# Storm-131/MARL-SortingEnv

Measured on AMD Instinct MI355X. Metric: env-steps/sec (random policy) Env_3_Monolith @65k envs, higher is better.
Workload: dtype int32+f64 (integer state/masks, fp64 rewards, f32 observations)

## Files before the change

__graft_entry__.py:

```python
from __future__ import annotations

import os
import sys

ROOT = os.path.dirname(os.path.abspath(__file__))
if ROOT not in sys.path:
    sys.path.insert(0, ROOT)


def build() -> None:
    import marl_sortingenv_amd as M

    path = M.build_library(force=False)
    assert os.path.exists(path), path
    from marl_sortingenv_amd.build import build_widetie_library

    wide = build_widetie_library()
    assert os.path.exists(wide), wide
    L = M.load_library()
    assert L.mse_version() == 200
    from oracle import oracle as O

    O.build()
    O.lib()
    print(f"built {path} and {O._SO}")


def smoke() -> None:
    import numpy as np
    import torch

    import marl_sortingenv_amd as M
    from oracle.oracle import OracleEnv

    assert torch.cuda.is_available(), "smoke() needs a GPU"
    n, K = 96, 24
    env = M.BatchedSortingEnv(kind="mono", num_envs=n, device=0, base_seed=11, max_steps=10, noise_sorting=0.05,
                              balesize=200, auto_reset=True)
    oracles = [OracleEnv(kind="mono", max_steps=10, seed=11 + i, noise_sorting=0.05, balesize=200) for i in range(n)]
    for i, o in enumerate(oracles):
        assert np.array_equal(env.obs[i].cpu().numpy(), o.reset(11 + i))
    buf = env.rollout(K, policy_seed=5)
    torch.cuda.synchronize()
    act, obs, rew = buf["actions"].cpu().numpy(), buf["obs"].cpu().numpy(), buf["reward"].cpu().numpy()
    done, mask = buf["done"].cpu().numpy(), buf["mask"].cpu().numpy()
    for k in range(K):
        for i, o in enumerate(oracles):
            assert o.action_masks()[act[k, i]] == 1
            eo, er, et = o.step(int(act[k, i]))
            if et:
                eo = o.reset(None)
            assert np.array_equal(eo.view(np.uint32), obs[k, i].view(np.uint32)), (k, i)
            assert abs(er - float(rew[k, i])) <= 1e-6 and bool(done[k, i]) == et
            assert np.array_equal(o.action_masks(), mask[k, i])
    print(f"smoke ok: {n} envs x {K} steps on {torch.cuda.get_device_name(0)} match the oracle "
          f"(lib: {M.library_path()})")


if __name__ == "__main__":
    build()
    if len(sys.argv) > 1 and sys.argv[1] == "smoke":
        smoke()
```

include/mse.h:

```cpp
#ifndef MSE_H
#define MSE_H

#include <stddef.h>
#include <stdint.h>

#ifdef __cplusplus
extern "C" {
#endif

#define MSE_VERSION 200

typedef enum mse_status {
    MSE_OK = 0,
    MSE_ERR_INVALID_ARGUMENT = -1,
    MSE_ERR_UNSUPPORTED_CONFIG = -2,
    MSE_ERR_NO_DEVICE = -3,
    MSE_ERR_HIP = -4,
    MSE_ERR_NOT_RESET = -5,
    MSE_ERR_ALIGNMENT = -6
} mse_status;

typedef enum mse_env_kind { MSE_ENV_SORT = 1, MSE_ENV_PRESS = 2, MSE_ENV_MONO = 3 } mse_env_kind;

#define MSE_STEP_UNMASKED       1u
// ... 66 lines not shown

int mse_rollout(mse_env *env, int32_t k_steps, uint64_t policy_seed, const int32_t *sort_mode_dev,
                uint32_t flags, int32_t *actions_out, float *obs_out, float *reward_out,
                uint8_t *done_out, uint8_t *mask_out, void *stream);

int mse_sample_actions(mse_env *env, uint64_t policy_seed, int32_t *action_out, void *stream);

int mse_rule_actions(mse_env *env, int32_t *action_out, void *stream);

#define MSE_SNAP_INTS 71
#define MSE_SNAP_RNG_WORDS 30
int mse_get_state(mse_env *env, int64_t *ints_out, double *dbls_out, uint64_t *rng_out, void *stream);
int mse_set_state(mse_env *env, const int64_t *ints_in, const double *dbls_in, const uint64_t *rng_in, void *stream);

int mse_model_actions(mse_env *env, uint32_t flags, int32_t *action_out, void *stream);

#define MSE_MODEL_PRESS_AGENT_MASKED 64u
struct mse_policy;
int mse_rollout_model(mse_env *env, struct mse_policy *sort_agent, struct mse_policy *press_agent, int32_t k_steps, uint32_t flags,
                      int32_t *actions_out, float *obs_out, float *reward_out, uint8_t *done_out, uint8_t *mask_out,
                      float *sort_obs_out, float *press_obs_out, void *stream);

#define MSE_TRACE_COLS       40
#define MSE_TRACE_ACTION      0
#define MSE_TRACE_R_SORT      1
#define MSE_TRACE_R_PRESS     2
#define MSE_TRACE_SETTING     3
#define MSE_TRACE_BELT        4
#define MSE_TRACE_CONT_TRUE   8
#define MSE_TRACE_CONT_FALSE 12
#define MSE_TRACE_CONT_E     16
#define MSE_TRACE_N_LOG      17
#define MSE_TRACE_LOG        18
#define MSE_TRACE_N_BALE     22
#define MSE_TRACE_BALE       23
#define MSE_TRACE_DONE       29
#define MSE_TRACE_STEP       30
#define MSE_TRACE_INTERNAL   31
#define MSE_TRACE_REWARD     32
#define MSE_TRACE_ACC_BELT   33
#define MSE_TRACE_OVERFLOW   37
int mse_trace_begin(mse_env *env, int64_t env_index, double *records_dev, int64_t capacity);
int mse_trace_end(mse_env *env, int64_t *n_records_out);

int mse_get_policy_step(const mse_env *env, uint64_t *t_out);
int mse_set_policy_step(mse_env *env, uint64_t t);

int mse_error_count(mse_env *env, uint64_t *count_out);

int mse_algorithmic_bytes_per_step(const mse_env *env);

uint32_t mse_tie_window(void);

typedef struct mse_policy mse_policy;
int64_t mse_policy_num_weights(int obs_dim, int n_actions);
int mse_policy_create(mse_policy **out, int obs_dim, int n_actions, const float *weights_host, int device_id);
int mse_policy_destroy(mse_policy *policy);
int mse_policy_set_precision(mse_policy *policy, int mode);
int mse_policy_precision(const mse_policy *policy);
int mse_policy_forward(mse_policy *policy, int64_t n, int64_t index_offset, const float *obs_dev, const uint8_t *mask_dev,
                       uint64_t seed, uint64_t t, int deterministic, int32_t *action_out, float *logp_out,
                       float *value_out, float *logits_out, void *stream);

int mse_rollout_policy(mse_env *env, mse_policy *policy, mse_policy *sort_policy, int32_t k_steps, uint64_t seed, int deterministic,
                       const int32_t *sort_mode_dev, uint32_t flags, float *obs_out, uint8_t *mask_out,
                       int32_t *actions_out, float *logp_out, float *value_out, float *reward_out,
                       uint8_t *episode_start_out, float *last_value_out, uint8_t *last_done_out, void *stream);

#define MSE_MODULAR_SORT_DETERMINISTIC  128u
#define MSE_MODULAR_PRESS_DETERMINISTIC 256u
typedef struct mse_modular_buffers {
    uint32_t struct_size;
    uint32_t reserved0;
    float   *sort_obs;
    float   *press_obs;
    uint8_t *press_masks;
    uint8_t *episode_starts;
    int32_t *sort_actions;
    int32_t *press_actions;
    float   *sort_log_probs;
    float   *press_log_probs;
    float   *sort_values;
    float   *press_values;
    float   *rewards;
    float   *rewards_sort;
    float   *rewards_press;
    float   *sort_last_values;
    float   *press_last_values;
    uint8_t *last_dones;
} mse_modular_buffers;
int mse_rollout_modular(mse_env *env, mse_policy *sort_agent, mse_policy *press_agent, int32_t k_steps, uint64_t sort_seed,
                        uint64_t press_seed, uint32_t flags, const mse_modular_buffers *out, void *stream);
int mse_rollout_modular_check(mse_env *env, mse_policy *sort_agent, mse_policy *press_agent, int32_t k_steps,
                              uint64_t sort_seed, uint64_t press_seed, uint32_t flags);

typedef struct mse_modular_label_buffers {
    uint32_t struct_size;
    uint32_t reserved0;
    int32_t *sort_expert_actions;
    int32_t *press_expert_actions;
    int32_t *stepped_actions;
    uint8_t *expert_stepped;
} mse_modular_label_buffers;
int mse_rollout_modular_labelled(mse_env *env, mse_policy *sort_agent, mse_policy *press_agent, int32_t k_steps,
                                 uint64_t sort_seed, uint64_t press_seed, uint64_t mix_seed, uint32_t expert_threshold,
                                 uint32_t flags, const mse_modular_buffers *out, const mse_modular_label_buffers *labels,
// ... 145 lines not shown
```

marl-sortingenv_amd/_lib.py:

```python
from __future__ import annotations

import ctypes as C
import os

from .build import LIB_PATH

MSE_ENV_SORT, MSE_ENV_PRESS, MSE_ENV_MONO = 1, 2, 3
MSE_STEP_UNMASKED, MSE_STEP_CHECK_OVERFLOW, MSE_ROLLOUT_RULE_BASED, MSE_STEP_SANITIZE_LATE = 1, 2, 4, 8
MSE_MODEL_NO_SORT_DRAW, MSE_MODEL_NO_PRESS_DRAW = 16, 32
MSE_MODEL_PRESS_AGENT_MASKED = 64
MSE_MODULAR_SORT_DETERMINISTIC, MSE_MODULAR_PRESS_DETERMINISTIC = 128, 256
MSE_DEMO_ACTOR_DETERMINISTIC = 512
MSE_PREVIEW_DETERMINISTIC = 1024
MSE_SNAP_INTS = 71
MSE_SNAP_RNG_WORDS = 30
MSE_TRACE_COLS = 40

EXPORTS = [
    "mse_version", "mse_last_error", "mse_status_string", "mse_config_default", "mse_create",
    "mse_create_indexed", "mse_destroy", "mse_num_envs", "mse_obs_dim", "mse_num_actions", "mse_reset",
    "mse_step", "mse_action_masks", "mse_rollout", "mse_sample_actions", "mse_rule_actions", "mse_get_state", "mse_set_state",
    "mse_error_count", "mse_algorithmic_bytes_per_step", "mse_tie_window",
    "mse_sort_agent_obs", "mse_policy_num_weights", "mse_policy_create", "mse_policy_destroy", "mse_policy_forward",
    "mse_get_policy_step", "mse_set_policy_step", "mse_model_actions", "mse_trace_begin", "mse_trace_end", "mse_press_agent_obs", "mse_rollout_policy", "mse_policy_set_precision", "mse_policy_precision",
    "mse_rollout_model", "mse_rollout_modular", "mse_rollout_modular_check",
    "mse_policy_set_weights", "mse_gae", "mse_ppo_workspace_bytes", "mse_ppo_loss_grad", "mse_ppo_adam_step",
    "mse_ppo_shuffle", "mse_ppo_shuffle_host",
    "mse_policy_set_weights_device", "mse_policy_sync", "mse_policy_image_floats", "mse_policy_pack_host",
    "mse_policy_read_image", "mse_policy_get_weights", "mse_ppo_loss_grad_gated", "mse_ppo_adam_step_gated",
    "mse_episode_workspace_bytes", "mse_episode_scan", "mse_episode_scan_host", "mse_episode_summary", "mse_episode_summary_host",
    "mse_ppo_loss_grad_matrix",
    "mse_ppo_loss_grad_vclip", "mse_explained_variance_workspace_bytes", "mse_explained_variance", "mse_explained_variance_host",
    "mse_bc_loss_grad", "mse_ppo_bc_workspace_bytes", "mse_ppo_bc_loss_grad",
    "mse_rollout_demo", "mse_rollout_demo_check", "mse_demo_who_steps_host",
    "mse_rollout_policy_labelled", "mse_rollout_policy_labelled_check",
    "mse_rollout_modular_labelled", "mse_rollout_modular_labelled_check",
    "mse_mono_agent_obs", "mse_rollout_policy_preview", "mse_rollout_policy_preview_check",
]

_other_libs: dict = {}


class MseError(RuntimeError):
    def __init__(self, status: int, message: str):
        super().__init__(f"libmse_hip status {status}: {message}")
        self.status = status


class MseConfigStruct(C.Structure):
    _fields_ = [
        ("struct_size", C.c_uint32), ("env_kind", C.c_int32), ("max_steps", C.c_int32),
        ("auto_reset", C.c_int32), ("track_bales", C.c_int32), ("literal_choice", C.c_int32),
        ("input_batch_size", C.c_int32), ("steps_per_pattern", C.c_int32),
        ("baseline_accuracy", C.c_double * 4), ("boost", C.c_double), ("noise", C.c_double),
        ("stage_capacity", C.c_int32),
        ("press_time", C.c_int32 * 2), ("container_capacity", C.c_int32), ("bale_standard_size", C.c_int32),
        ("bale_remainder_threshold", C.c_double), ("quality_threshold", C.c_double * 4),
        ("quality_threshold_r2", C.c_double * 4),
        ("purity_threshold_theta", C.c_double), ("tanh_temperature", C.c_double),
        ("overflow_penalty_catastrophic", C.c_double), ("overflow_penalty_severe", C.c_double),
        ("overflow_penalty_mild", C.c_double), ("bale_efficiency_factor", C.c_double),
        ("max_state_reward", C.c_double), ("overflow_termination_penalty", C.c_double),
        ("pattern_ratio", (C.c_double * 4) * 2),
        ("rollout_pipeline", C.c_int32), ("reserved0", C.c_int32),
    ]


class MsePpoParams(C.Structure):
    _fields_ = [("struct_size", C.c_uint32), ("clip_range", C.c_float), ("ent_coef", C.c_float), ("vf_coef", C.c_float),
                ("normalize_advantage", C.c_int32)]


MODULAR_BUFFER_NAMES = ("sort_obs", "press_obs", "press_masks", "episode_starts", "sort_actions", "press_actions",
                        "sort_log_probs", "press_log_probs", "sort_values", "press_values", "rewards", "rewards_sort",
                        "rewards_press", "sort_last_values", "press_last_values", "last_dones")
# ... 150 lines not shown
```

marl-sortingenv_amd/build.py:

```python
from __future__ import annotations

import os
import shutil
import subprocess

PKG_DIR = os.path.dirname(os.path.abspath(__file__))
REPO_ROOT = os.path.dirname(PKG_DIR)
SOURCES = [os.path.join(PKG_DIR, "csrc", "mse_lib.hip"), os.path.join(PKG_DIR, "csrc", "mse_policy.hip"),
           os.path.join(PKG_DIR, "csrc", "mse_ppo.hip"), os.path.join(PKG_DIR, "csrc", "mse_ppo_matrix.hip"),
           os.path.join(PKG_DIR, "csrc", "mse_episode.hip")]
HEADERS = [os.path.join(PKG_DIR, "csrc", h) for h in ("mse_device.h", "mse_exact.h", "mse_host.h", "mse_params.h", "mse_plan.h", "mse_tables.h", "mse_policy_device.h", "mse_policy_pack.h", "mse_policy_stream.h", "mse_demo_mix.h", "mse_ppo_math.h", "mse_ppo_grad.h", "mse_ppo_grad_body.inc", "mse_ppo_matrix_body.inc", "mse_rollout_policy_body.inc", "mse_rollout_modular_body.inc", "mse_plain_frame.inc", "mse_episode_math.h")] + \
          [os.path.join(REPO_ROOT, "include", "mse.h")]
LIB_PATH = os.environ.get("MSE_LIB_PATH") or os.path.join(PKG_DIR, "libmse_hip.so")

HIPCC_FLAGS = [
    "-O3", "--offload-arch=gfx950", "-std=c++17", "-fPIC", "-shared",
    "-ffp-contract=off", "-fno-fast-math",
]


def hipcc_path() -> str:
    for cand in (shutil.which("hipcc"), "/opt/rocm/bin/hipcc"):
        if cand and os.path.exists(cand):
            return cand
    raise RuntimeError("hipcc not found: libmse_hip.so cannot be built")


def is_stale() -> bool:
    if not os.path.exists(LIB_PATH):
        return True
    t = os.path.getmtime(LIB_PATH)
    return any(os.path.getmtime(p) > t for p in SOURCES + HEADERS)


def build_library(force: bool = False, verbose: bool = False) -> str:
    if not force and not is_stale():
        return LIB_PATH
    cmd = [hipcc_path(), *HIPCC_FLAGS, "-I", os.path.join(REPO_ROOT, "include"), *SOURCES, "-o", LIB_PATH]
    if verbose:
        print(" ".join(cmd))
    subprocess.run(cmd, check=True)
    return LIB_PATH


WIDETIE_LIB_PATH = os.path.join(PKG_DIR, "libmse_hip_widetie.so")


def build_widetie_library(force: bool = False) -> str:
    if not force and os.path.exists(WIDETIE_LIB_PATH) and \
            all(os.path.getmtime(p) <= os.path.getmtime(WIDETIE_LIB_PATH) for p in SOURCES + HEADERS):
        return WIDETIE_LIB_PATH
    cmd = [hipcc_path(), *HIPCC_FLAGS, "-DMSE_TIE_WINDOW=0x08000000u", "-I", os.path.join(REPO_ROOT, "include"),
           *SOURCES, "-o", WIDETIE_LIB_PATH]
    subprocess.run(cmd, check=True)
    return WIDETIE_LIB_PATH


if __name__ == "__main__":
    print(build_widetie_library(force=True))
    print(build_library(force=True, verbose=True))
```

marl-sortingenv_amd/csrc/mse_device.h:

```cpp
#pragma once

#include <hip/hip_runtime.h>
#include <stdint.h>

#include "mse_exact.h"
#include "mse_params.h"
#include "mse_policy_stream.h"

namespace mse {

constexpr int kGeneratorPeriod = 20;

enum Plane : int {
    PL_RNG_STATE = 0,
    PL_RNG_INC,
    PL_ACC01,
    PL_ACC23,
    PL_CONT_TRUE,
    PL_CONT_FALSE,
    PL_MISC0,
    PL_MISC1,
    PL_MISC2,
    PL_NOISE_STATE,
    PL_NOISE_INC,
// ... 143 lines not shown
        hb *= MULT_B;
        v *= hb;
        v ^= v >> 16;
        st[i] = v;
    }
#pragma unroll
    for (int i = 0; i < 4; ++i) out[i] = (uint64_t)st[2 * i] | ((uint64_t)st[2 * i + 1] << 32);
}

__device__ inline Pcg pcg_seed(uint64_t seed)
{
    uint64_t w[4];
    seed_sequence(seed, w);
    Pcg g;
    g.i_hi = (w[2] << 1) | (w[3] >> 63);
    g.i_lo = (w[3] << 1) | 1ull;
    g.s_lo = 0;
    g.s_hi = 0;
    pcg_advance(g);
    uint64_t lo = g.s_lo + w[1];
    g.s_hi = g.s_hi + w[0] + (lo < g.s_lo ? 1ull : 0ull);
    g.s_lo = lo;
    pcg_advance(g);
    return g;
}

__device__ __forceinline__ uint64_t mix64(uint64_t z)
{
    z = (z ^ (z >> 30)) * 0xBF58476D1CE4E5B9ull;
    z = (z ^ (z >> 27)) * 0x94D049BB133111EBull;
    return z ^ (z >> 31);
}

__device__ __forceinline__ int select_kth_bit(uint32_t bits, int k)
{
    uint32_t lo = bits & 0x7FFu;
    int c = __popc(lo);
    bool up = k >= c;
    k = up ? k - c : k;
    bits = up ? bits >> 11 : lo;
    int base = up ? 11 : 0;
    lo = bits & 0x3Fu;
    c = __popc(lo);
    up = k >= c;
    k = up ? k - c : k;
    bits = up ? bits >> 6 : lo;
    base += up ? 6 : 0;
    for (int i = 0; i < k; ++i) bits &= bits - 1u;
    return base + __ffs((int)bits) - 1;
}

#ifdef MSE_TIMELINE
__device__ unsigned long long g_timeline[4 * 8];
struct Timeline {
    unsigned long long last;
    unsigned long long acc[8];
    __device__ __forceinline__ void start()
    {
        for (int k = 0; k < 8; ++k) acc[k] = 0;
        last = __builtin_readcyclecounter();
    }
    __device__ __forceinline__ void mark(int k)
    {
        if (blockIdx.x != 0) return;
        const unsigned long long now = __builtin_readcyclecounter();
        acc[k] += now - last;
        last = now;
    }
    __device__ __forceinline__ void flush(int role) const
    {
        if ((threadIdx.x & 63) == 0 && blockIdx.x == 0)
            for (int k = 0; k < 8; ++k) atomicAdd(&g_timeline[role * 8 + k], acc[k]);
    }
};
#if MSE_TIMELINE == 2
#define MSE_TL(tl, k) ((void)0)
#define MSE_TLB(tl, k) (tl).mark(k)
#else
#define MSE_TL(tl, k) (tl).mark(k)
#define MSE_TLB(tl, k) (tl).mark(k)
#endif
#else
#define MSE_TLB(tl, k) ((void)0)
#define MSE_TL(tl, k) ((void)0)
#endif

struct Env {
#ifdef MSE_TIMELINE
    Timeline tl;
#endif
    Pcg rng;
    Pcg noise;
    Pcg press;
    uint32_t press_uint;
    int press_has;
    Pcg gen;
    uint32_t gen_uint;
    int gen_has;
    double acc[4];
    int ct[4], cf[4], ce;
    int pn[2], lpa;
    int st_in, st_belt, st_sort;
    int timer[2], pmat[2], q100[2];
    int mode, lps, gen2, gen_idx, gen_cnt, step;
    uint32_t episode;
};

__device__ __forceinline__ int stage_id(uint32_t word, const Params &P)
{
    if (P.gen_mode) return (int)word;
    return word == 0u ? 0 : (word == P.pat_word[1] ? 1 : 2);
}
__device__ __forceinline__ uint32_t stage_word(int id, const Params &P)
{
    if (P.gen_mode) return (uint32_t)id;
    return id == 0 ? P.pat_word[0] : (id == 1 ? P.pat_word[1] : P.pat_word[2]);
}

struct EnvRaw {
    uint4 a, b, c0, c1, t, f, m0, m1, m2, ns, nq, ps, pq;
};

template <int KIND, bool NOISE>
__device__ __forceinline__ void load_env_raw(EnvRaw &r, const uint4 *__restrict__ planes, const Params &P, long long i)
{
    const long long n_pad = P.n_pad;
    r.a = planes[PL_RNG_STATE * n_pad + i];
    r.b = planes[PL_RNG_INC * n_pad + i];
    r.c0 = planes[PL_ACC01 * n_pad + i];
    r.c1 = planes[PL_ACC23 * n_pad + i];
    r.t = planes[PL_CONT_TRUE * n_pad + i];
    r.f = planes[PL_CONT_FALSE * n_pad + i];
    r.m0 = planes[PL_MISC0 * n_pad + i];
    r.m1 = planes[PL_MISC1 * n_pad + i];
    r.m2 = planes[PL_MISC2 * n_pad + i];
    if (NOISE) {
        r.ns = planes[PL_NOISE_STATE * n_pad + i];
// ... 1625 lines not shown
```

marl-sortingenv_amd/csrc/mse_lib.hip:

```cpp
#include "mse_device.h"
#include "mse_demo_mix.h"
#include "mse_host.h"
#include "mse_plan.h"
#include "mse_policy_device.h"
#include "mse_tables.h"

#include "mse.h"

#include <cmath>
#include <cstdio>
#include <cstdlib>
#include <cstring>
#include <memory>
#include <new>
#include <string>
#include <type_traits>
#include <vector>

using namespace mse;

extern __shared__ uint4 mse_dyn_lds[];

template <int KIND>
struct LdsLayout {
    static constexpr int D = Dims<KIND>::D, A = Dims<KIND>::A;
    static constexpr int obs_bytes = kBlock * D * 4;
    static constexpr int mask_bytes = (kBlock * A + 15) / 16 * 16;
    static constexpr int bale_offset = obs_bytes + mask_bytes;
    static constexpr int bale_bytes = 5 * kBlock * 16;
    static constexpr int table_offset_step = bale_offset;
    static constexpr int table_offset_rollout = bale_offset + bale_bytes;
};

__device__ __forceinline__ void lds_barrier_all()
{
    asm volatile("s_waitcnt lgkmcnt(0)\n\ts_barrier" ::: "memory");
}

template <int THREADS, int U>
struct TableCopy {
    uint4 x[U];
    __device__ __forceinline__ void issue(const uint32_t *__restrict__ src, int words, int t)
    {
        const uint4 *s4 = reinterpret_cast<const uint4 *>(src);
        const int n4 = words >> 2;
#pragma unroll
        for (int u = 0; u < U; ++u) {
            const int idx = u * THREADS + t;
            x[u] = s4[idx < n4 ? idx : n4 - 1];
        }
    }
    __device__ __forceinline__ void commit(uint32_t *dst, const uint32_t *__restrict__ src, int words, int t) const
    {
        uint4 *d4 = reinterpret_cast<uint4 *>(dst);
        const uint4 *s4 = reinterpret_cast<const uint4 *>(src);
        const int n4 = words >> 2;
#pragma unroll
        for (int u = 0; u < U; ++u) {
            const int idx = u * THREADS + t;
            if (idx < n4) d4[idx] = x[u];
        }
        for (int idx = U * THREADS + t; idx < n4; idx += THREADS) d4[idx] = s4[idx];
    }
};

__device__ __forceinline__ void load_tables_to_lds(uint32_t *dst, const uint32_t *__restrict__ src, int words, int tid)
{
    TableCopy<kBlock, 4> tc;
    tc.issue(src, words, tid);
    tc.commit(dst, src, words, tid);
    __syncthreads();
}

typedef float nt_f32x4 __attribute__((ext_vector_type(4)));
typedef unsigned int nt_u32x4 __attribute__((ext_vector_type(4)));
__device__ __forceinline__ void store_stream(float4 *p, const float4 &v)
{
    nt_f32x4 x = {v.x, v.y, v.z, v.w};
    __builtin_nontemporal_store(x, reinterpret_cast<nt_f32x4 *>(p));
}
__device__ __forceinline__ void store_stream(uint4 *p, const uint4 &v)
{
    nt_u32x4 x = {v.x, v.y, v.z, v.w};
    __builtin_nontemporal_store(x, reinterpret_cast<nt_u32x4 *>(p));
}

typedef uint32_t u32_align2 __attribute__((aligned(2)));
template <int A, class P16>
__device__ __forceinline__ void write_mask_row(P16 *row16, uint32_t mbits)
// ... 465 lines not shown
            Snap sn;
#pragma unroll
            for (int m = 0; m < 4; ++m) {
                sn.ct[m] = (int)w[(kSnapCt + m) * kPoEnvs];
                sn.cf[m] = (int)w[(kSnapCf + m) * kPoEnvs];
            }
            sn.ce = (int)w[kSnapCe * kPoEnvs];
            sn.lpa = (int)w[kSnapLpa * kPoEnvs];
            const uint32_t pk = w[kSnapStatus * kPoEnvs];
            const int a = (int)w[kSnapAction * kPoEnvs];
            const uint32_t mbits = w[kSnapMask * kPoEnvs];
            if (NOISE) {
#pragma unroll
                for (int m = 0; m < 4; ++m)
                    sn.acc[m] = __hiloint2double((int)w[(kSnapAcc + 2 * m + 1) * kPoEnvs], (int)w[(kSnapAcc + 2 * m) * kPoEnvs]);
            }
            unpack_snap_status(pk, sn);
            if (live) {
                int k[4];
                StepResult r = env_observe<KIND, NOISE>(sn, P, tb, k, o);
                if (__builtin_expect(sn.done != 0, 0)) {
                    Snap rs;
                    snap_of_reset(rs, tb.cst);
                    int k2[4];
                    (void)env_observe<KIND, true>(rs, P, tb, k2, o);
                }
                if (actions_out != nullptr) __builtin_nontemporal_store(a, &actions_out[(long long)s * P.n + i]);
                if (reward_out != nullptr) __builtin_nontemporal_store((float)r.reward, &reward_out[(long long)s * P.n + i]);
                if (done_out != nullptr) __builtin_nontemporal_store((uint8_t)r.done, &done_out[(long long)s * P.n + i]);
            }
            const long long srow = (long long)s * P.n + row0;
            stage_and_store<KIND>(lds, L::obs_bytes, o, mbits, obs_out ? obs_out + srow * D : nullptr,
                                  mask_out ? mask_out + srow * A : nullptr, n_valid_block, tid - kPoEnvs);
        }
    }
}

constexpr int kRingThreads = 3 * kPoEnvs;

template <int KIND, bool NOISE>
struct RingLayout {
    static constexpr int D = Dims<KIND>::D, A = Dims<KIND>::A;
    static constexpr int snap_words = snap_word_count(NOISE, false);
    static constexpr int ring_offset = 0;
    static constexpr int ring_bytes = kRingDepth * kPoEnvs * 4;
    static_assert(ring_bytes == 65536, "RngRing::load assumes 64 rows of 1 KiB");
    static constexpr int stage_offset = ring_bytes;
    static constexpr int stage_bytes = kPoEnvs * D * 4;
    static constexpr int snap_offset = stage_offset + stage_bytes;
    static constexpr int snap_bytes = 2 * snap_words * kPoEnvs * 4;
    static constexpr int bale_offset = snap_offset + snap_bytes;
    static constexpr int bale_bytes = 5 * kPoEnvs * 16;
    static constexpr int pos_offset = bale_offset + bale_bytes;
    static constexpr int pos_bytes = kPoEnvs * 4;
    static constexpr int table_offset = pos_offset + pos_bytes;
};

__device__ __forceinline__ void rng_server_role(const Params &P, uint4 *__restrict__ planes, const Tables &tb, long long i,
                                                bool live, int k_steps, uint32_t *lring, uint32_t *lpos, int el, bool two_halves,
                                                int barriers_before_init = 0)
{
    Pcg g = Pcg::from_planes(planes[PL_RNG_STATE * P.n_pad + i], planes[PL_RNG_INC * P.n_pad + i]);
    const uint32_t ring_lane_addr = (uint32_t)(uintptr_t)(__attribute__((address_space(3))) uint32_t *)(lring + el);
    uint64_t c2_lo, c2_hi;
    mul128(0x4385DF649FCCF646ull, 0x2360ED051FC65DA4ull, g.i_lo, g.i_hi, c2_lo, c2_hi);
    const uint32_t worst = (uint32_t)P.ring_worst;
    uint32_t w = 0, need = worst, cap = need;
#ifdef MSE_TIMELINE
    Timeline tl;
    tl.start();
#endif
    for (int s = -1; s < k_steps; ++s) {
        const uint32_t deficit = need > w ? need - w : 0u;
        uint32_t M = 0;
#pragma unroll
        for (int bit = 5; bit >= 0; --bit) {
            const uint32_t cand = M | (1u << bit);
            if (__builtin_amdgcn_ballot_w64(deficit >= cand) != 0ull) M = cand;
        }
        const uint32_t room = cap > w ? cap - w : 0u;
#ifdef MSE_TIMELINE
        if (blockIdx.x == 0) {
            tl.acc[3] += M;
            unsigned long long produced = 0;
            for (int b = 0; b < 6; ++b) produced += ((unsigned long long)__builtin_popcountll(__builtin_amdgcn_ballot_w64((((M < room ? M : room) >> b) & 1u) != 0))) << b;
            tl.acc[4] += produced;
        }
#endif
#ifdef MSE_ABL_NORNG
        w += M < room ? M : room;
#else
        {
            const uint32_t count = M < room ? M : room;
            ring_produce_pairs(g, w, count >> 1, ring_lane_addr, c2_lo, c2_hi);
            ring_produce(g, w, count & 1u, ring_lane_addr);
        }
#endif
        MSE_TLB(tl, 0);
        if (s < 0)
            for (int b = 0; b < barriers_before_init; ++b) lds_barrier_all();
        lds_barrier_all();
        MSE_TLB(tl, 1);
        if (s < 0 && two_halves) {
            pcg_affine(g, P.ring_fwd[0], P.ring_fwd[1], P.ring_fwd[2], P.ring_fwd[3]);
            w += worst;
        }
        const uint32_t steps_left = (uint32_t)(k_steps - 1 - s);
        const uint32_t r = lpos[el];
        const uint32_t ahead = worst * steps_left;
        need = r + worst * (steps_left < 2u ? steps_left : 2u);
        cap = r + (ahead < (uint32_t)kRingDepth ? ahead : (uint32_t)kRingDepth);
    }
    {
        uint32_t d = w - lpos[el];
        if (__builtin_expect(d > 32u, 0)) {
            pcg_step_back(g, 32u, tb.back);
            d -= 32u;
        }
        pcg_step_back(g, d, tb.back);
        if (live) planes[PL_RNG_STATE * P.n_pad + i] = pack_u64x2(g.s_lo, g.s_hi);
    }
#ifdef MSE_TIMELINE
    tl.flush(2);
#endif
}

constexpr int kRingTwoHalvesFrom = 16;

#ifdef MSE_CLOCK_PROBE
__device__ unsigned long long g_clock_probe[3];
__device__ unsigned long long g_wg_probe[3 * 1024];
#endif
template <int KIND, bool NOISE>
__global__ __launch_bounds__(kRingThreads) void k_rollout_ring(Params P, uint4 *__restrict__ planes,
                                                               const uint32_t *__restrict__ table_image, int k_steps,
                                                               uint64_t policy_seed, uint64_t policy_t0,
                                                               const int *__restrict__ sort_mode, uint32_t flags,
                                                               int *__restrict__ actions_out,
                                                               float *__restrict__ obs_out,
                                                               float *__restrict__ reward_out,
                                                               uint8_t *__restrict__ done_out,
                                                               uint8_t *__restrict__ mask_out)
{
    using L = RingLayout<KIND, NOISE>;
    constexpr int D = L::D, A = L::A, SW = L::snap_words;
    uint8_t *lds = reinterpret_cast<uint8_t *>(mse_dyn_lds);
    uint32_t *ltab = reinterpret_cast<uint32_t *>(lds + L::table_offset);
    uint32_t *lsnap = reinterpret_cast<uint32_t *>(lds + L::snap_offset);
    uint4 *lbale = reinterpret_cast<uint4 *>(lds + L::bale_offset);
    uint32_t *lring = reinterpret_cast<uint32_t *>(lds + L::ring_offset);
    uint32_t *lpos = reinterpret_cast<uint32_t *>(lds + L::pos_offset);
    const int tid = threadIdx.x;
    const int role = tid / kPoEnvs;
    const int el = tid - role * kPoEnvs;
    const long long row0 = (long long)blockIdx.x * kPoEnvs;
    const bool live = row0 + el < P.n;
    const long long i = live ? row0 + el : P.n - 1;
#ifdef MSE_TIMELINE
    Timeline edge;
    edge.start();
#endif
#ifdef MSE_CLOCK_PROBE
    const unsigned long long probe_c0 = __builtin_readcyclecounter(), probe_r0 = __builtin_amdgcn_s_memrealtime();
#endif

    const Tables tb = tables_at(ltab, P);
    Env e;
    EnvRaw raw;
    int sm = -1;
    if (role == 0) {
        load_env_raw<KIND, NOISE>(raw, planes, P, i);
        if (KIND == 2 && sort_mode != nullptr) sm = sort_mode[i];
    }
    if (role == 0) {
        TableCopy<2 * kPoEnvs, 2> tc;
        tc.issue(table_image, P.table_words, tid);
        tc.commit(ltab, table_image, P.table_words, tid);
        unpack_env<KIND, NOISE>(e, raw, P);
    } else if (role == 1) {
        uint4 ps = {}, pi = {};
        const bool two_halves = k_steps >= kRingTwoHalvesFrom;
        if (two_halves) {
            ps = planes[PL_RNG_STATE * P.n_pad + i];
            pi = planes[PL_RNG_INC * P.n_pad + i];
        }
        TableCopy<2 * kPoEnvs, 2> tc;
        tc.issue(table_image, P.table_words, tid);
        if (two_halves) {
            Pcg g;
            g.s_lo = (uint64_t)ps.x | ((uint64_t)ps.y << 32);
            g.s_hi = (uint64_t)ps.z | ((uint64_t)ps.w << 32);
            g.i_lo = (uint64_t)pi.x | ((uint64_t)pi.y << 32);
            g.i_hi = (uint64_t)pi.z | ((uint64_t)pi.w << 32);
            pcg_affine(g, P.ring_fwd[0], P.ring_fwd[1], P.ring_fwd[2], P.ring_fwd[3]);
            uint32_t w2 = (uint32_t)P.ring_worst;
            ring_produce(g, w2, (uint32_t)P.ring_worst,
                         (uint32_t)(uintptr_t)(__attribute__((address_space(3))) uint32_t *)(lring + el));
        }
        tc.commit(ltab, table_image, P.table_words, tid);
    }
    MSE_TL(edge, 0);

    if (role == 2) {
        rng_server_role(P, planes, tb, i, live, k_steps, lring, lpos, el, k_steps >= kRingTwoHalvesFrom);
    } else if (role == 0) {
        __builtin_amdgcn_s_setprio(3);
        const BaleRef bales{lbale + el, kPoEnvs};
        if (P.track_bales) {
#pragma unroll
            for (int m = 0; m < 5; ++m) lbale[m * kPoEnvs + el] = planes[(long long)(PL_BALE0 + m) * P.n_pad + i];
        }
        __builtin_amdgcn_s_waitcnt(0x0F70);
        RngRing rng;
        rng.open(lring, el, tb.jump, e);
        uint32_t cur_mask = action_mask_bits<KIND>(e, P);
        const uint32_t pkey = mse_policy_key(policy_seed, (uint64_t)(P.index_offset + i));
        lpos[el] = 0;
        MSE_TL(edge, 1);
        lds_barrier_all();
        MSE_TL(edge, 2);
#ifdef MSE_TIMELINE
        e.tl.start();
#endif
        for (int s = 0; s < k_steps; ++s) {
            {
                const int a = policy_action<KIND>(e, cur_mask, tb, flags, pkey, policy_t0 + (uint64_t)s);
                MSE_TL(e.tl, 0);
                Snap sn;
                env_dynamics<KIND, NOISE, false>(e, rng, P, tb, a, sm, flags, bales, sn);
                uint32_t *w = lsnap + (s & 1) * SW * kPoEnvs + el;
#pragma unroll
                for (int m = 0; m < 4; ++m) {
                    w[(kSnapCt + m) * kPoEnvs] = (uint32_t)sn.ct[m];
                    w[(kSnapCf + m) * kPoEnvs] = (uint32_t)sn.cf[m];
                }
                w[kSnapCe * kPoEnvs] = (uint32_t)sn.ce;
                w[kSnapLpa * kPoEnvs] = (uint32_t)sn.lpa;
                w[kSnapStatus * kPoEnvs] = pack_snap_status(sn);
                w[kSnapAction * kPoEnvs] = (uint32_t)a;
                if (NOISE) {
#pragma unroll
                    for (int m = 0; m < 4; ++m) w[(kSnapAcc + m) * kPoEnvs] = __float_as_uint((float)sn.acc[m]);
                }
                if (__builtin_expect(sn.done != 0, 0)) {
                    int kdummy[4];
                    auto_reset_env(e, P, tb, bales, kdummy);
                }
                const uint32_t mbits = action_mask_bits<KIND>(e, P);
                cur_mask = mbits;
                w[kSnapMask * kPoEnvs] = mbits;
                lpos[el] = rng.pos();
            }
            MSE_TLB(e.tl, 5);
            lds_barrier_all();
            MSE_TLB(e.tl, 6);
        }
#ifdef MSE_TIMELINE
        e.tl.flush(0);
#endif
        MSE_TL(edge, 3);
        if (live) {
            store_env<KIND, NOISE>(e, planes, P, i, false, false);
        }
        if (P.track_bales && live) {
#pragma unroll
            for (int m = 0; m < 5; ++m) planes[(long long)(PL_BALE0 + m) * P.n_pad + i] = lbale[m * kPoEnvs + el];
        }
        MSE_TL(edge, 5);
#ifdef MSE_TIMELINE
        edge.flush(3);
#endif
    } else {
        long long rem = P.n - row0;
        const int n_valid_block = rem >= kPoEnvs ? kPoEnvs : (rem > 0 ? (int)rem : 0);
        float o[D];
#pragma unroll
        for (int j = 0; j < D; ++j) o[j] = 0.0f;
        lds_barrier_all();
#ifdef MSE_TIMELINE
        Timeline tl;
        tl.start();
#endif
        for (int s = 0; s < k_steps; ++s) {
            lds_barrier_all();
            MSE_TLB(tl, 0);
            const uint32_t *w = lsnap + (s & 1) * SW * kPoEnvs + el;
            Snap sn;
#pragma unroll
            for (int m = 0; m < 4; ++m) {
                sn.ct[m] = (int)w[(kSnapCt + m) * kPoEnvs];
                sn.cf[m] = (int)w[(kSnapCf + m) * kPoEnvs];
            }
            sn.ce = (int)w[kSnapCe * kPoEnvs];
            sn.lpa = (int)w[kSnapLpa * kPoEnvs];
            const uint32_t pk = w[kSnapStatus * kPoEnvs];
            const int a = (int)w[kSnapAction * kPoEnvs];
            const uint32_t mbits = w[kSnapMask * kPoEnvs];
            if (NOISE) {
#pragma unroll
                for (int m = 0; m < 4; ++m) sn.acc[m] = (double)__uint_as_float(w[(kSnapAcc + m) * kPoEnvs]);
            }
            unpack_snap_status(pk, sn);
            int k[4];
#ifdef MSE_ABL_NOOBS
            StepResult r{0.0, sn.done, 0.0, 0.0};
#else
            StepResult r = env_observe<KIND, NOISE>(sn, P, tb, k, o);
#endif
            if (__builtin_expect(sn.done != 0, 0)) {
                Snap rs;
                snap_of_reset(rs, tb.cst);
                int k2[4];
                (void)env_observe<KIND, true>(rs, P, tb, k2, o);
            }
            if (live) {
                if (actions_out != nullptr) __builtin_nontemporal_store(a, &actions_out[(long long)s * P.n + i]);
                if (reward_out != nullptr) __builtin_nontemporal_store((float)r.reward, &reward_out[(long long)s * P.n + i]);
                if (done_out != nullptr) __builtin_nontemporal_store((uint8_t)r.done, &done_out[(long long)s * P.n + i]);
            }
            MSE_TL(tl, 1);
            const long long srow = (long long)s * P.n + row0;
            {
            stage_and_store<KIND>(lds + L::stage_offset, -1, o, mbits, obs_out ? obs_out + srow * D : nullptr, nullptr, n_valid_block,
                                  tid - kPoEnvs);
            stage_and_store<KIND>(lds + L::stage_offset, -1, o, mbits, nullptr, mask_out ? mask_out + srow * A : nullptr, n_valid_block,
                                  tid - kPoEnvs);
            }
            MSE_TLB(tl, 2);
        }
#ifdef MSE_TIMELINE
        tl.flush(1);
#endif
    }
#ifdef MSE_CLOCK_PROBE
    if (tid == kPoEnvs && blockIdx.x == 0) {
        atomicAdd(&g_clock_probe[0], __builtin_readcyclecounter() - probe_c0);
        atomicAdd(&g_clock_probe[1], __builtin_amdgcn_s_memrealtime() - probe_r0);
        atomicAdd(&g_clock_probe[2], 1ull);
    }
    if (tid == kPoEnvs && blockIdx.x < 1024) {
        g_wg_probe[3 * blockIdx.x] = probe_r0;
        g_wg_probe[3 * blockIdx.x + 1] = __builtin_amdgcn_s_memrealtime();
        g_wg_probe[3 * blockIdx.x + 2] = (unsigned long long)__builtin_amdgcn_s_getreg(((4 - 1) << 11) | (0 << 6) | 20);
    }
#endif
}


template <int KIND, int TILES>
struct PolLayout {
    static constexpr int kind = KIND, D = Dims<KIND>::D, A = Dims<KIND>::A;
    static constexpr int ENVS = 32 * TILES;
    static constexpr int weight_bytes = msep::kLdsFloats * 4;
    static constexpr int tile_bytes = (ENVS * D * 4 + 15) / 16 * 16;
    static constexpr int bale_bytes = 5 * ENVS * 16;
    static constexpr int wave_bytes = tile_bytes + bale_bytes;
};

typedef __attribute__((address_space(3))) float lds_f32;
typedef __attribute__((address_space(3))) uint16_t lds_u16;
__device__ __forceinline__ uint32_t lds_row_address(const void *row)
{
    uint32_t a = (uint32_t)(uintptr_t)(__attribute__((address_space(3))) const void *)row;
    asm volatile("" : "+v"(a));
    return a;
}

template <int D, int ROWS>
__device__ __forceinline__ void wave_tile_to_global_f32(const float *ltile, float *g, int n_valid, int lane)
{
    constexpr int NQ = ROWS * D / 4;
    if (n_valid == ROWS && (reinterpret_cast<uintptr_t>(g) & 15u) == 0) {
        const float4 *src = reinterpret_cast<const float4 *>(ltile);
        float4 *dst = reinterpret_cast<float4 *>(g);
        constexpr int NR = (NQ + 63) / 64;
        float4 buf[NR];
#pragma unroll
        for (int j = 0; j < NR; ++j) buf[j] = src[(lane + 64 * j) < NQ ? lane + 64 * j : 0];
#pragma unroll
        for (int j = 0; j < NR; ++j)
            if (lane + 64 * j < NQ) store_stream(dst + lane + 64 * j, buf[j]);
    } else {
        for (int q = lane; q < n_valid * D; q += 64) g[q] = ltile[q];
    }
}
template <int D, int ROWS>
__device__ __forceinline__ void wave_store_rows_f32(float *ltile, uint32_t lrow, const float *o, float *g, int n_valid, int lane)
{
    if (lane < ROWS) {
        lds_f32 *row = (lds_f32 *)(uintptr_t)lrow;
#pragma unroll
        for (int j = 0; j < D; ++j) row[j] = o[j];
    }
    __builtin_amdgcn_wave_barrier();
    wave_tile_to_global_f32<D, ROWS>(ltile, g, n_valid, lane);
// ... 1288 lines not shown
template <int KIND>
static void launch_rollout_demo(mse_env *h, const mse_policy *actor, hipStream_t s, int k_steps, uint64_t seed,
                                uint64_t mix_seed, uint32_t expert_threshold, uint32_t flags, const mse_demo_buffers &out)
{
    const PolicyPlan plan = plan_rollout_demo<KIND>(h, actor);
    with_flags([&](auto NOISE, auto ONE_TILE, auto F16, auto ACTOR) {
        if constexpr ((F16 || !ONE_TILE) && (ACTOR || F16))
            hipLaunchKernelGGL((k_rollout_demo<KIND, NOISE, ONE_TILE ? 1 : 2, F16, ACTOR>), dim3((unsigned)plan.workgroups),
                               dim3((unsigned)(64 * plan.n_waves)), plan.lds_bytes, s, h->P, h->planes, h->tables,
                               actor != nullptr ? actor->blob : nullptr, k_steps, seed, mix_seed, expert_threshold,
                               h->policy_t, flags, out);
    }, h->noise_on, plan.tiles == 1, actor == nullptr || actor->use_f16(), actor != nullptr);
}

static PolicyPlan plan_rollout_policy_preview(const mse_env *h, const mse_policy *pol)
{
    return plan_policy_plain(h->P.n, h->cus, pol->use_f16(), 1, policy_lds<3>(h->P));
}

static void launch_rollout_policy_preview(mse_env *h, const mse_policy *pol, hipStream_t s, int k_steps, uint64_t seed,
                                          uint64_t mix_seed, uint32_t expert_threshold, uint32_t flags,
                                          const mse_preview_buffers &out)
{
    const PolicyPlan plan = plan_rollout_policy_preview(h, pol);
    with_flags([&](auto NOISE, auto ONE_TILE, auto F16) {
        if constexpr (F16 || !ONE_TILE)
            hipLaunchKernelGGL((k_rollout_policy_preview<NOISE, ONE_TILE ? 1 : 2, F16>), dim3((unsigned)plan.workgroups),
                               dim3((unsigned)(64 * plan.n_waves)), plan.lds_bytes, s, h->P, h->planes, h->tables, pol->blob,
                               k_steps, seed, mix_seed, expert_threshold, h->policy_t, flags, out);
    }, h->noise_on, plan.tiles == 1, pol->use_f16());
}

static int rollout_checks(const mse_env *h, int32_t k_steps, const char *fn)
{
    if (!h) return fail(MSE_ERR_INVALID_ARGUMENT, "env is NULL");
    if (!h->seeded) return fail(MSE_ERR_NOT_RESET, std::string(fn) + " before mse_reset(seeds)");
    if (k_steps < 1) return fail(MSE_ERR_INVALID_ARGUMENT, "k_steps must be >= 1");
    if (!h->P.auto_reset) return fail(MSE_ERR_INVALID_ARGUMENT, std::string(fn) + " needs auto_reset=1");
    if (h->trace_rec != nullptr)
        return fail(MSE_ERR_INVALID_ARGUMENT, "a trace is attached (mse_trace_begin): only mse_step records, end it first");
    return MSE_OK;
}

static int integer_path_check(const mse_env *h, const char *fn, const char *advice)
{
    if (!h->literal && !h->P.gen_mode) return MSE_OK;
    return fail(MSE_ERR_UNSUPPORTED_CONFIG, std::string(fn) + " serves the integer draw path with a remainder-free batch (" + advice + ")");
}

extern "C" {

int mse_version(void) { return MSE_VERSION; }
uint32_t mse_tie_window(void) { return MSE_TIE_WINDOW; }
#ifdef MSE_CLOCK_PROBE
int mse_debug_clock(unsigned long long *out3)
{
    unsigned long long zero[3] = {};
    if (hipDeviceSynchronize() != hipSuccess) return -1;
    if (hipMemcpyFromSymbol(out3, HIP_SYMBOL(g_clock_probe), sizeof(zero)) != hipSuccess) return -1;
    if (hipMemcpyToSymbol(HIP_SYMBOL(g_clock_probe), zero, sizeof(zero)) != hipSuccess) return -1;
    return 0;
}
int mse_debug_wg_probe(unsigned long long *out3072)
{
    if (hipDeviceSynchronize() != hipSuccess) return -1;
    return hipMemcpyFromSymbol(out3072, HIP_SYMBOL(g_wg_probe), sizeof(unsigned long long) * 3 * 1024) == hipSuccess ? 0 : -1;
}
#endif
#ifdef MSE_TIMELINE
int mse_debug_timeline(unsigned long long *out32)
{
    unsigned long long zero[32] = {};
    if (hipDeviceSynchronize() != hipSuccess) return -1;
    if (hipMemcpyFromSymbol(out32, HIP_SYMBOL(mse::g_timeline), sizeof(zero)) != hipSuccess) return -1;
    if (hipMemcpyToSymbol(HIP_SYMBOL(mse::g_timeline), zero, sizeof(zero)) != hipSuccess) return -1;
    return 0;
}
#endif

const char *mse_last_error(void) { return g_last_error.c_str(); }
}
int mse_internal_fail(int status, const char *msg) { return fail(status, msg); }
extern "C" {

const char *mse_status_string(int status)
{
    switch (status) {
    case MSE_OK: return "ok";
    case MSE_ERR_INVALID_ARGUMENT: return "invalid argument";
    case MSE_ERR_UNSUPPORTED_CONFIG: return "unsupported configuration";
    case MSE_ERR_NO_DEVICE: return "no HIP device";
    case MSE_ERR_HIP: return "HIP runtime error";
    case MSE_ERR_NOT_RESET: return "mse_reset with seeds has not run yet";
    case MSE_ERR_ALIGNMENT: return "buffer not 16-byte aligned";
    default: return "unknown status";
    }
}

int mse_config_default(mse_config *c)
{
    if (!c) return fail(MSE_ERR_INVALID_ARGUMENT, "cfg is NULL");
    std::memset(c, 0, sizeof(*c));
    c->struct_size = (uint32_t)sizeof(mse_config);
    c->env_kind = MSE_ENV_MONO;
    c->max_steps = 50;
    c->auto_reset = 1;
    c->track_bales = 1;
    c->literal_choice = 0;
    c->input_batch_size = 100;
    c->steps_per_pattern = 20;
    for (int m = 0; m < 4; ++m) {
        c->baseline_accuracy[m] = 0.75;
        c->quality_threshold[m] = 0.9;
        c->quality_threshold_r2[m] = 0.9;
    }
    c->boost = 0.5;
    c->noise = 0.05;
    c->stage_capacity = 100;
    c->press_time[0] = 12;
    c->press_time[1] = 15;
    c->container_capacity = 700;
    c->bale_standard_size = 200;
// ... 619 lines not shown
```

Baseline: 20.66 billion.

## Replace workgroup barriers with per-wave LDS counter handoffs between ring roles

```diff
diff --git a/__graft_entry__.py b/__graft_entry__.py
--- a/__graft_entry__.py
+++ b/__graft_entry__.py
@@ -17,6 +17,10 @@
 
     wide = build_widetie_library()
     assert os.path.exists(wide), wide
+    from marl_sortingenv_amd.build import build_wgbarrier_library
+
+    wgb = build_wgbarrier_library()
+    assert os.path.exists(wgb), wgb
     L = M.load_library()
     assert L.mse_version() == 200
     from oracle import oracle as O
diff --git a/include/mse.h b/include/mse.h
--- a/include/mse.h
+++ b/include/mse.h
@@ -142,6 +142,8 @@
 
 uint32_t mse_tie_window(void);
 
+int mse_ring_handoff(void);
+
 typedef struct mse_policy mse_policy;
 int64_t mse_policy_num_weights(int obs_dim, int n_actions);
 int mse_policy_create(mse_policy **out, int obs_dim, int n_actions, const float *weights_host, int device_id);
diff --git a/marl-sortingenv_amd/_lib.py b/marl-sortingenv_amd/_lib.py
--- a/marl-sortingenv_amd/_lib.py
+++ b/marl-sortingenv_amd/_lib.py
@@ -20,7 +20,7 @@
     "mse_version", "mse_last_error", "mse_status_string", "mse_config_default", "mse_create",
     "mse_create_indexed", "mse_destroy", "mse_num_envs", "mse_obs_dim", "mse_num_actions", "mse_reset",
     "mse_step", "mse_action_masks", "mse_rollout", "mse_sample_actions", "mse_rule_actions", "mse_get_state", "mse_set_state",
-    "mse_error_count", "mse_algorithmic_bytes_per_step", "mse_tie_window",
+    "mse_error_count", "mse_algorithmic_bytes_per_step", "mse_tie_window", "mse_ring_handoff",
     "mse_sort_agent_obs", "mse_policy_num_weights", "mse_policy_create", "mse_policy_destroy", "mse_policy_forward",
     "mse_get_policy_step", "mse_set_policy_step", "mse_model_actions", "mse_trace_begin", "mse_trace_end", "mse_press_agent_obs", "mse_rollout_policy", "mse_policy_set_precision", "mse_policy_precision",
     "mse_rollout_model", "mse_rollout_modular", "mse_rollout_modular_check",
diff --git a/marl-sortingenv_amd/build.py b/marl-sortingenv_amd/build.py
--- a/marl-sortingenv_amd/build.py
+++ b/marl-sortingenv_amd/build.py
@@ -56,6 +56,20 @@
     return WIDETIE_LIB_PATH
 
 
+WGBARRIER_LIB_PATH = os.path.join(PKG_DIR, "libmse_hip_wgbarrier.so")
+
+
+def build_wgbarrier_library(force: bool = False) -> str:
+    if not force and os.path.exists(WGBARRIER_LIB_PATH) and \
+            all(os.path.getmtime(p) <= os.path.getmtime(WGBARRIER_LIB_PATH) for p in SOURCES + HEADERS):
+        return WGBARRIER_LIB_PATH
+    cmd = [hipcc_path(), *HIPCC_FLAGS, "-DMSE_RING_WG_BARRIER", "-I", os.path.join(REPO_ROOT, "include"),
+           *SOURCES, "-o", WGBARRIER_LIB_PATH]
+    subprocess.run(cmd, check=True)
+    return WGBARRIER_LIB_PATH
+
+
 if __name__ == "__main__":
     print(build_widetie_library(force=True))
+    print(build_wgbarrier_library(force=True))
     print(build_library(force=True, verbose=True))
diff --git a/marl-sortingenv_amd/csrc/mse_device.h b/marl-sortingenv_amd/csrc/mse_device.h
--- a/marl-sortingenv_amd/csrc/mse_device.h
+++ b/marl-sortingenv_amd/csrc/mse_device.h
@@ -219,6 +219,8 @@
 
 #ifdef MSE_TIMELINE
 __device__ unsigned long long g_timeline[4 * 8];
+constexpr int kTimelineStampSteps = 64;
+__device__ unsigned long long g_timeline_stamp[12 * kTimelineStampSteps * 2];
 struct Timeline {
     unsigned long long last;
     unsigned long long acc[8];
@@ -238,6 +240,11 @@
     {
         if ((threadIdx.x & 63) == 0 && blockIdx.x == 0)
             for (int k = 0; k < 8; ++k) atomicAdd(&g_timeline[role * 8 + k], acc[k]);
+    }
+    __device__ __forceinline__ void stamp(int s, int which) const
+    {
+        if (blockIdx.x == 0 && (threadIdx.x & 63) == 0 && s < kTimelineStampSteps)
+            g_timeline_stamp[((threadIdx.x >> 6) * kTimelineStampSteps + s) * 2 + which] = last;
     }
 };
 #if MSE_TIMELINE == 2
@@ -247,9 +254,11 @@
 #define MSE_TL(tl, k) (tl).mark(k)
 #define MSE_TLB(tl, k) (tl).mark(k)
 #endif
+#define MSE_TLS(tl, s, which) (tl).stamp(s, which)
 #else
 #define MSE_TLB(tl, k) ((void)0)
 #define MSE_TL(tl, k) ((void)0)
+#define MSE_TLS(tl, s, which) ((void)0)
 #endif
 
 struct Env {
diff --git a/marl-sortingenv_amd/csrc/mse_lib.hip b/marl-sortingenv_amd/csrc/mse_lib.hip
--- a/marl-sortingenv_amd/csrc/mse_lib.hip
+++ b/marl-sortingenv_amd/csrc/mse_lib.hip
@@ -35,6 +35,40 @@
 __device__ __forceinline__ void lds_barrier_all()
 {
     asm volatile("s_waitcnt lgkmcnt(0)\n\ts_barrier" ::: "memory");
+}
+
+__device__ __forceinline__ void hand_publish(uint32_t *ctr, uint32_t count)
+{
+    const uint32_t addr = (uint32_t)(uintptr_t)(__attribute__((address_space(3))) uint32_t *)ctr;
+    uint64_t saved;
+    asm volatile(
+#ifdef MSE_RING_HAND_DRAIN
+                 "s_waitcnt lgkmcnt(0)\n\t"
+#endif
+                 "s_mov_b64 %0, exec\n\t"
+                 "s_mov_b64 exec, 1\n\t"
+                 "ds_write_b32 %1, %2\n\t"
+                 "s_mov_b64 exec, %0"
+                 : "=&s"(saved)
+                 : "v"(addr), "v"(count)
+                 : "memory");
+}
+__device__ __forceinline__ void hand_wait(const uint32_t *ctr, uint32_t at_least)
+{
+    const uint32_t addr = (uint32_t)(uintptr_t)(__attribute__((address_space(3))) const uint32_t *)ctr;
+    uint32_t seen_v, seen_s;
+    asm volatile("1:\n\t"
+                 "ds_read_b32 %0, %2\n\t"
+                 "s_waitcnt lgkmcnt(0)\n\t"
+                 "v_readfirstlane_b32 %1, %0\n\t"
+                 "s_cmp_ge_u32 %1, %3\n\t"
+                 "s_cbranch_scc1 2f\n\t"
+                 "s_sleep 1\n\t"
+                 "s_branch 1b\n"
+                 "2:"
+                 : "=&v"(seen_v), "=&s"(seen_s)
+                 : "v"(addr), "s"(at_least)
+                 : "memory", "scc");
 }
 
 template <int THREADS, int U>
@@ -606,13 +640,23 @@
     static constexpr int bale_offset = snap_offset + snap_bytes;
     static constexpr int bale_bytes = 5 * kPoEnvs * 16;
     static constexpr int pos_offset = bale_offset + bale_bytes;
+#ifdef MSE_RING_WG_BARRIER
     static constexpr int pos_bytes = kPoEnvs * 4;
-    static constexpr int table_offset = pos_offset + pos_bytes;
+    static constexpr int hand_bytes = 0;
+#else
+    static constexpr int pos_bytes = 2 * kPoEnvs * 4;
+    static constexpr int hand_bytes = 64;
+#endif
+    static constexpr int hand_offset = pos_offset + pos_bytes;
+    static constexpr int table_offset = hand_offset + hand_bytes;
 };
 
+constexpr int kHandDyn = 0, kHandObs = 4, kHandRng = 8;
+
+template <bool HAND = false>
 __device__ __forceinline__ void rng_server_role(const Params &P, uint4 *__restrict__ planes, const Tables &tb, long long i,
                                                 bool live, int k_steps, uint32_t *lring, uint32_t *lpos, int el, bool two_halves,
-                                                int barriers_before_init = 0)
+                                                int barriers_before_init = 0, uint32_t *hand = nullptr)
 {
     Pcg g = Pcg::from_planes(planes[PL_RNG_STATE * P.n_pad + i], planes[PL_RNG_INC * P.n_pad + i]);
     const uint32_t ring_lane_addr = (uint32_t)(uintptr_t)(__attribute__((address_space(3))) uint32_t *)(lring + el);
@@ -651,22 +695,29 @@
         }
 #endif
         MSE_TLB(tl, 0);
+        if (barriers_before_init == 0 && s >= 0) MSE_TLS(tl, s, 0);
         if (s < 0)
             for (int b = 0; b < barriers_before_init; ++b) lds_barrier_all();
-        lds_barrier_all();
+        if (HAND && s >= 0) {
+            hand_publish(hand + kHandRng, (uint32_t)s + 1u);
+            hand_wait(hand + kHandDyn, (uint32_t)s + 1u);
+        } else {
+            lds_barrier_all();
+        }
         MSE_TLB(tl, 1);
+        if (barriers_before_init == 0 && s >= 0) MSE_TLS(tl, s, 1);
         if (s < 0 && two_halves) {
             pcg_affine(g, P.ring_fwd[0], P.ring_fwd[1], P.ring_fwd[2], P.ring_fwd[3]);
             w += worst;
         }
         const uint32_t steps_left = (uint32_t)(k_steps - 1 - s);
-        const uint32_t r = lpos[el];
+        const uint32_t r = lpos[HAND ? (s & 1) * kPoEnvs + el : el];
         const uint32_t ahead = worst * steps_left;
         need = r + worst * (steps_left < 2u ? steps_left : 2u);
         cap = r + (ahead < (uint32_t)kRingDepth ? ahead : (uint32_t)kRingDepth);
     }
     {
-        uint32_t d = w - lpos[el];
+        uint32_t d = w - lpos[HAND ? ((k_steps - 1) & 1) * kPoEnvs + el : el];
         if (__builtin_expect(d > 32u, 0)) {
             pcg_step_back(g, 32u, tb.back);
             d -= 32u;
@@ -710,6 +761,15 @@
     const long long row0 = (long long)blockIdx.x * kPoEnvs;
     const bool live = row0 + el < P.n;
     const long long i = live ? row0 + el : P.n - 1;
+#ifdef MSE_RING_WG_BARRIER
+    constexpr bool kHand = false;
+    constexpr int kPosStride = 0;
+    uint32_t *const hand = nullptr;
+#else
+    constexpr bool kHand = true;
+    constexpr int kPosStride = kPoEnvs;
+    uint32_t *const hand = reinterpret_cast<uint32_t *>(lds + L::hand_offset) + (el >> 6);
+#endif
 #ifdef MSE_TIMELINE
     Timeline edge;
     edge.start();
@@ -756,7 +816,7 @@
     MSE_TL(edge, 0);
 
     if (role == 2) {
-        rng_server_role(P, planes, tb, i, live, k_steps, lring, lpos, el, k_steps >= kRingTwoHalvesFrom);
+        rng_server_role<kHand>(P, planes, tb, i, live, k_steps, lring, lpos, el, k_steps >= kRingTwoHalvesFrom, 0, hand);
     } else if (role == 0) {
         __builtin_amdgcn_s_setprio(3);
         const BaleRef bales{lbale + el, kPoEnvs};
@@ -770,6 +830,10 @@
         uint32_t cur_mask = action_mask_bits<KIND>(e, P);
         const uint32_t pkey = mse_policy_key(policy_seed, (uint64_t)(P.index_offset + i));
         lpos[el] = 0;
+        if (kHand) {
+            lpos[kPosStride + el] = 0;
+            if ((el & 63) < 3) hand[4 * (el & 63)] = 0u;
+        }
         MSE_TL(edge, 1);
         lds_barrier_all();
         MSE_TL(edge, 2);
@@ -783,6 +847,7 @@
                 Snap sn;
                 env_dynamics<KIND, NOISE, false>(e, rng, P, tb, a, sm, flags, bales, sn);
                 uint32_t *w = lsnap + (s & 1) * SW * kPoEnvs + el;
+                if (kHand && s >= 2) hand_wait(hand + kHandObs, (uint32_t)s - 1u);
 #pragma unroll
                 for (int m = 0; m < 4; ++m) {
                     w[(kSnapCt + m) * kPoEnvs] = (uint32_t)sn.ct[m];
@@ -803,11 +868,18 @@
                 const uint32_t mbits = action_mask_bits<KIND>(e, P);
                 cur_mask = mbits;
                 w[kSnapMask * kPoEnvs] = mbits;
-                lpos[el] = rng.pos();
+                lpos[(s & 1) * kPosStride + el] = rng.pos();
             }
             MSE_TLB(e.tl, 5);
-            lds_barrier_all();
+            MSE_TLS(e.tl, s, 0);
+            if (kHand) {
+                hand_publish(hand + kHandDyn, (uint32_t)s + 1u);
+                if (s + 1 < k_steps) hand_wait(hand + kHandRng, (uint32_t)s + 1u);
+            } else {
+                lds_barrier_all();
+            }
             MSE_TLB(e.tl, 6);
+            MSE_TLS(e.tl, s, 1);
         }
 #ifdef MSE_TIMELINE
         e.tl.flush(0);
@@ -836,8 +908,11 @@
         tl.start();
 #endif
         for (int s = 0; s < k_steps; ++s) {
-            lds_barrier_all();
+            MSE_TLS(tl, s, 0);
+            if (kHand) hand_wait(hand + kHandDyn, (uint32_t)s + 1u);
+            else lds_barrier_all();
             MSE_TLB(tl, 0);
+            MSE_TLS(tl, s, 1);
             const uint32_t *w = lsnap + (s & 1) * SW * kPoEnvs + el;
             Snap sn;
 #pragma unroll
@@ -854,6 +929,7 @@
 #pragma unroll
                 for (int m = 0; m < 4; ++m) sn.acc[m] = (double)__uint_as_float(w[(kSnapAcc + m) * kPoEnvs]);
             }
+            if (kHand) hand_publish(hand + kHandObs, (uint32_t)s + 1u);
             unpack_snap_status(pk, sn);
             int k[4];
 #ifdef MSE_ABL_NOOBS
@@ -892,9 +968,9 @@
         atomicAdd(&g_clock_probe[1], __builtin_amdgcn_s_memrealtime() - probe_r0);
         atomicAdd(&g_clock_probe[2], 1ull);
     }
+    if (role == 1 && (tid & 63) == 0 && blockIdx.x < 1024) atomicMax(&g_wg_probe[3 * blockIdx.x + 1], __builtin_amdgcn_s_memrealtime());
     if (tid == kPoEnvs && blockIdx.x < 1024) {
         g_wg_probe[3 * blockIdx.x] = probe_r0;
-        g_wg_probe[3 * blockIdx.x + 1] = __builtin_amdgcn_s_memrealtime();
         g_wg_probe[3 * blockIdx.x + 2] = (unsigned long long)__builtin_amdgcn_s_getreg(((4 - 1) << 11) | (0 << 6) | 20);
     }
 #endif
@@ -2289,6 +2365,14 @@
 
 int mse_version(void) { return MSE_VERSION; }
 uint32_t mse_tie_window(void) { return MSE_TIE_WINDOW; }
+int mse_ring_handoff(void)
+{
+#ifdef MSE_RING_WG_BARRIER
+    return 0;
+#else
+    return 1;
+#endif
+}
 #ifdef MSE_CLOCK_PROBE
 int mse_debug_clock(unsigned long long *out3)
 {
@@ -2305,6 +2389,11 @@
 }
 #endif
 #ifdef MSE_TIMELINE
+int mse_debug_timeline_stamps(unsigned long long *out1536)
+{
+    if (hipDeviceSynchronize() != hipSuccess) return -1;
+    return hipMemcpyFromSymbol(out1536, HIP_SYMBOL(mse::g_timeline_stamp), sizeof(unsigned long long) * 12 * 64 * 2) == hipSuccess ? 0 : -1;
+}
 int mse_debug_timeline(unsigned long long *out32)
 {
     unsigned long long zero[32] = {};
```

Result: no change. 20.66 billion (-0.0%).
